# BDMstudio/audio-cut

Measured on AMD Instinct MI355X. Metric: audio-seconds processed/sec (separate+detect) per GPU; cut-point index parity, higher is better.
Workload: dtype f32

## Files before the change

### audio_cut_amd/csrc/ac_mdx.hip

```cpp
#include <math.h>

#include "ac_common.h"
#include "../../include/audiocut_hip_stereo.h"

#define MDX_NFFT 6144
#define MDX_M 3072
#define MDX_HOP 1024
#define MDX_T 256
#define MDX_F 3072
#define MDX_ITEM 261120
#define MDX_TRIM 3072
#define MDX_GEN 254976

__device__ inline float2 cmulf(float2 a, float2 b) { return make_float2(a.x * b.x - a.y * b.y, a.x * b.y + a.y * b.x); }

__device__ inline float2 tw3072(const float2* __restrict__ tw, int q) {
    int k = 2 * q;
    if (k >= MDX_M) { const float2 t = tw[k - MDX_M]; return make_float2(-t.x, -t.y); }
    return tw[k];
}

__device__ float2* fft3072_f32(float2* a, float2* b, const float2* __restrict__ tw) {
    int Ns = 1;
    for (int pass = 0; pass < 5; ++pass) {
        for (int j = threadIdx.x; j < MDX_M / 4; j += 256) {
            const int k = j & (Ns - 1);
            float2 v0 = a[j], v1 = a[j + MDX_M / 4], v2 = a[j + MDX_M / 2], v3 = a[j + 3 * MDX_M / 4];
            if (Ns > 1) {
                const int q = k * (MDX_M / (4 * Ns));
                v1 = cmulf(v1, tw3072(tw, q));
                v2 = cmulf(v2, tw3072(tw, 2 * q));
                v3 = cmulf(v3, tw3072(tw, 3 * q));
            }
            const float2 s02 = make_float2(v0.x + v2.x, v0.y + v2.y), d02 = make_float2(v0.x - v2.x, v0.y - v2.y);
            const float2 s13 = make_float2(v1.x + v3.x, v1.y + v3.y), d13 = make_float2(v1.x - v3.x, v1.y - v3.y);
            const int base = ((j - k) << 2) + k;
            b[base] = make_float2(s02.x + s13.x, s02.y + s13.y);
            b[base + Ns] = make_float2(d02.x + d13.y, d02.y - d13.x);
            b[base + 2 * Ns] = make_float2(s02.x - s13.x, s02.y - s13.y);
            b[base + 3 * Ns] = make_float2(d02.x - d13.y, d02.y + d13.x);
        }
        __syncthreads();
        float2* t = a; a = b; b = t;
        Ns <<= 2;
    }
    {
        const float c3 = -0.5f, s3 = -0.86602540378443864676f;
        for (int j = threadIdx.x; j < MDX_M / 3; j += 256) {
            const int k = j;
            float2 v0 = a[j], v1 = a[j + 1024], v2 = a[j + 2048];
            v1 = cmulf(v1, tw3072(tw, k));
            v2 = cmulf(v2, tw3072(tw, 2 * k));
            const float2 s = make_float2(v1.x + v2.x, v1.y + v2.y);
            const float2 d = make_float2(v1.x - v2.x, v1.y - v2.y);
            const float2 m = make_float2(v0.x + c3 * s.x, v0.y + c3 * s.y);
            const float2 r = make_float2(-s3 * d.y, s3 * d.x);
            b[k] = make_float2(v0.x + s.x, v0.y + s.y);
            b[k + 1024] = make_float2(m.x + r.x, m.y + r.y);
            b[k + 2048] = make_float2(m.x - r.x, m.y - r.y);
        }
        __syncthreads();
        float2* t = a; a = b; b = t;
    }
    return a;
}

template <int CH>
__global__ __launch_bounds__(256) void k_mdx_stft(const float* __restrict__ track, int64_t n,
                                                  const int64_t* __restrict__ chunk_start,
                                                  const int64_t* __restrict__ chunk_len,
                                                  const int32_t* __restrict__ win_index,
                                                  const float2* __restrict__ tw, const float* __restrict__ hann,
                                                  float* __restrict__ spec, float* __restrict__ spec_amax) {
    __shared__ float2 s_a[MDX_M];
    __shared__ float2 s_b[MDX_M];
    const int t = blockIdx.x;
    const int item = blockIdx.y;
    const int ch = CH == 2 ? (int)blockIdx.z : 0;
    const float* x = track + (size_t)ch * n;
    const int64_t cs = chunk_start[item];
    const int64_t cl = chunk_len[item];
    const int64_t woff = (int64_t)win_index[item] * MDX_GEN - MDX_TRIM;
    for (int m = threadIdx.x; m < MDX_M; m += 256) {
        float v[2];
#pragma unroll
        for (int h = 0; h < 2; ++h) {
            const int i = 2 * m + h;
            int jj = t * MDX_HOP - MDX_NFFT / 2 + i;
            if (jj < 0) jj = -jj;
            else if (jj >= MDX_ITEM) jj = 2 * (MDX_ITEM - 1) - jj;
            const int64_t q = woff + jj;
            const float s = (q >= 0 && q < cl) ? x[cs + q] : 0.f;
            v[h] = s * hann[i];
        }
        s_a[m] = make_float2(v[0], v[1]);
    }
    __syncthreads();
    const float2* Z = fft3072_f32(s_a, s_b, tw);
    const size_t cstride = (size_t)MDX_T * MDX_F;
    float* out = spec + (size_t)item * 4 * cstride + 2 * ch * cstride + (size_t)t * MDX_F;
    float vmax = 0.f;
    for (int k = threadIdx.x; k < MDX_F; k += 256) {
        const float2 zk = Z[k];
        const float2 zn = Z[(MDX_M - k) % MDX_M];
        const float2 e = make_float2(0.5f * (zk.x + zn.x), 0.5f * (zk.y - zn.y));
        const float2 o = make_float2(0.5f * (zk.x - zn.x), 0.5f * (zk.y + zn.y));
        const float2 wo = cmulf(tw[k], o);
        const float re = e.x + wo.y, im = e.y - wo.x;
        out[k] = re;
        out[cstride + k] = im;
        if (CH == 1) {
            out[2 * cstride + k] = re;
            out[3 * cstride + k] = im;
        }
        vmax = fmaxf(vmax, fmaxf(fabsf(re), fabsf(im)));
    }
    if (spec_amax) ac_amax_commit(vmax, spec_amax + (size_t)item * MDX_T + t);
}

extern "C" int ac_mdx_stft(ac_ctx* ctx, const float* track, int64_t n, const int64_t* chunk_start, const int64_t* chunk_len,
                           const int32_t* win_index, int n_items, float* spec_out, float* spec_amax, void* stream) {
    AC_REQUIRE(ctx && track && chunk_start && chunk_len && win_index && spec_out, "null pointer");
    AC_REQUIRE(n > 0 && n_items > 0 && n_items <= 65535, "n_items must be in [1, 65535]");
    hipLaunchKernelGGL(k_mdx_stft<1>, dim3(MDX_T, n_items), dim3(256), 0, (hipStream_t)stream, track, n, chunk_start, chunk_len,
                       win_index, ctx->tw6144, ctx->hann6144, spec_out, spec_amax);
    AC_LAUNCH_CHECK();
    return AC_OK;
}

extern "C" int ac_mdx_stft_stereo(ac_ctx* ctx, const float* track, int64_t n, const int64_t* chunk_start, const int64_t* chunk_len,
                                  const int32_t* win_index, int n_items, float* spec_out, float* spec_amax, void* stream) {
    AC_REQUIRE(ctx && track && chunk_start && chunk_len && win_index && spec_out, "null pointer");
    AC_REQUIRE(n > 0 && n_items > 0 && n_items <= 65535, "n_items must be in [1, 65535]");
    hipLaunchKernelGGL(k_mdx_stft<2>, dim3(MDX_T, n_items, 2), dim3(256), 0, (hipStream_t)stream, track, n, chunk_start, chunk_len,
                       win_index, ctx->tw6144, ctx->hann6144, spec_out, spec_amax);
    AC_LAUNCH_CHECK();
    return AC_OK;
}

__global__ __launch_bounds__(256) void k_mdx_istft_frames(const float* __restrict__ spec, const float2* __restrict__ tw,
                                                          const float* __restrict__ hann, float* __restrict__ frames) {
    __shared__ float2 s_a[MDX_M];
    __shared__ float2 s_b[MDX_M];
    const int t = blockIdx.x, ch = blockIdx.y, item = blockIdx.z;
    const size_t cstride = (size_t)MDX_T * MDX_F;
    const float* re_p = spec + ((size_t)item * 4 + 2 * ch) * cstride + (size_t)t * MDX_F;
    const float* im_p = re_p + cstride;
    for (int k = threadIdx.x; k < MDX_M; k += 256) {
        float2 xk = make_float2(re_p[k], k == 0 ? 0.f : im_p[k]);
        float2 xm = (k == 0) ? make_float2(0.f, 0.f) : make_float2(re_p[MDX_M - k], im_p[MDX_M - k]);
        const float2 e = make_float2(0.5f * (xk.x + xm.x), 0.5f * (xk.y - xm.y));
        const float2 d = make_float2(0.5f * (xk.x - xm.x), 0.5f * (xk.y + xm.y));
        const float2 w = tw[k];
        const float2 o = cmulf(make_float2(w.x, -w.y), d);
        s_a[k] = make_float2(e.x - o.y, -(e.y + o.x));
    }
    __syncthreads();
    const float2* z = fft3072_f32(s_a, s_b, tw);
    const float inv = 1.0f / (float)MDX_M;
    float* out = frames + (((size_t)item * 2 + ch) * MDX_T + t) * MDX_NFFT;
    for (int m = threadIdx.x; m < MDX_M; m += 256) {
        const float2 v = z[m];
        const float x0 = v.x * inv, x1 = -v.y * inv;
        const float2 hw = reinterpret_cast<const float2*>(hann)[m];
        reinterpret_cast<float2*>(out)[m] = make_float2(x0 * hw.x, x1 * hw.y);
    }
}

__global__ __launch_bounds__(256) void k_mdx_istft_ola(const float* __restrict__ frames, const float* __restrict__ env,
                                                       float* __restrict__ wave) {
    const int64_t idx = (int64_t)blockIdx.x * 256 + threadIdx.x;
    const int64_t row = idx / MDX_ITEM;
    const int nn = (int)(idx - row * MDX_ITEM);
    const int p = nn + MDX_NFFT / 2;
    int t_lo = (p - (MDX_NFFT - 1) + MDX_HOP - 1) / MDX_HOP;
    if (p - (MDX_NFFT - 1) <= 0) t_lo = 0;
    int t_hi = p / MDX_HOP;
    if (t_hi > MDX_T - 1) t_hi = MDX_T - 1;
    const float* base = frames + (size_t)row * MDX_T * MDX_NFFT;
    float acc = 0.f;
    for (int t = t_lo; t <= t_hi; ++t) acc += base[(size_t)t * MDX_NFFT + (p - t * MDX_HOP)];
    wave[idx] = acc / env[p];
}

extern "C" int ac_mdx_istft(ac_ctx* ctx, const float* spec, int n_items, float* wave_out, float* scratch, void* stream) {
    AC_REQUIRE(ctx && spec && wave_out && scratch, "null pointer");
    AC_REQUIRE(n_items > 0 && n_items <= 65535, "n_items must be in [1, 65535]");
    hipLaunchKernelGGL(k_mdx_istft_frames, dim3(MDX_T, 2, n_items), dim3(256), 0, (hipStream_t)stream, spec, ctx->tw6144,
                       ctx->hann6144, scratch);
    AC_LAUNCH_CHECK();
    const int64_t total = (int64_t)n_items * 2 * MDX_ITEM;
    hipLaunchKernelGGL(k_mdx_istft_ola, dim3((unsigned)(total / 256)), dim3(256), 0, (hipStream_t)stream, scratch,
                       ctx->ola_env6144, wave_out);
    AC_LAUNCH_CHECK();
    return AC_OK;
}

template <int CH>
__global__ __launch_bounds__(256) void k_mdx_assemble_ola(const float* __restrict__ track, int64_t n, const float* __restrict__ wave,
                                                          const int64_t* __restrict__ chunk_start,
                                                          const int64_t* __restrict__ chunk_len,
                                                          const int64_t* __restrict__ eff_start,
                                                          const int64_t* __restrict__ eff_end,
                                                          const int32_t* __restrict__ item_base, int n_chunks,
                                                          float* __restrict__ vocal_out, float* __restrict__ inst_out,
                                                          float* __restrict__ vocal_st_out, float* __restrict__ inst_st_out) {
    const int64_t g = (int64_t)blockIdx.x * 256 + threadIdx.x;
    if (g >= n) return;
    int lo = 0, hi = n_chunks;
    while (lo < hi) { const int mid = (lo + hi) >> 1; if (eff_end[mid] > g) hi = mid; else lo = mid + 1; }
    const int c_lo = lo;
    const float m0 = track[g];
    const float m1 = CH == 2 ? track[n + g] : m0;
    float v_acc = 0.f, i_acc = 0.f, w_acc = 0.f;
    float v0_acc = 0.f, v1_acc = 0.f, i0_acc = 0.f, i1_acc = 0.f;
    for (int c = c_lo; c < n_chunks && eff_start[c] <= g; ++c) {
        if (eff_end[c] <= g) continue;
        const int64_t q = g - chunk_start[c];
        if (q < 0 || q >= chunk_len[c]) continue;
        const int item = item_base[c] + (int)(q / MDX_GEN);
        const int pos = MDX_TRIM + (int)(q % MDX_GEN);
        const float w0 = wave[((size_t)item * 2 + 0) * MDX_ITEM + pos];
        const float w1 = wave[((size_t)item * 2 + 1) * MDX_ITEM + pos];
        const float vocal = (w0 + w1) * 0.5f;
        const float inst = ((m0 - w0) + (m1 - w1)) * 0.5f;
        v_acc += vocal;
        i_acc += inst;
        w_acc += 1.0f;
        if (CH == 2) {
            v0_acc += w0; v1_acc += w1;
            i0_acc += m0 - w0; i1_acc += m1 - w1;
        }
    }
    if (w_acc == 0.f) w_acc = 1.0f;
    vocal_out[g] = v_acc / w_acc;
    inst_out[g] = i_acc / w_acc;
    if (CH == 2) {
        if (vocal_st_out) { vocal_st_out[g] = v0_acc / w_acc; vocal_st_out[n + g] = v1_acc / w_acc; }
        if (inst_st_out) { inst_st_out[g] = i0_acc / w_acc; inst_st_out[n + g] = i1_acc / w_acc; }
    }
}

extern "C" int ac_mdx_assemble_ola(ac_ctx* ctx, const float* track, int64_t n, const float* wave, const int64_t* chunk_start,
                                   const int64_t* chunk_len, const int64_t* eff_start, const int64_t* eff_end,
                                   const int32_t* item_base, int n_chunks, float* vocal_out, float* inst_out, void* stream) {
    AC_REQUIRE(ctx && track && wave && chunk_start && chunk_len && eff_start && eff_end && item_base && vocal_out && inst_out,
               "null pointer");
    AC_REQUIRE(n > 0 && n_chunks > 0, "sizes must be positive");
    const int64_t blocks = (n + 255) / 256;
    AC_REQUIRE(blocks < (1LL << 31), "track too long");
    hipLaunchKernelGGL(k_mdx_assemble_ola<1>, dim3((unsigned)blocks), dim3(256), 0, (hipStream_t)stream, track, n, wave, chunk_start,
                       chunk_len, eff_start, eff_end, item_base, n_chunks, vocal_out, inst_out, nullptr, nullptr);
    AC_LAUNCH_CHECK();
    return AC_OK;
}

extern "C" int ac_mdx_assemble_ola_stereo(ac_ctx* ctx, const float* track, int64_t n, const float* wave, const int64_t* chunk_start,
                                          const int64_t* chunk_len, const int64_t* eff_start, const int64_t* eff_end,
                                          const int32_t* item_base, int n_chunks, float* vocal_out, float* inst_out,
                                          float* vocal_st_out, float* inst_st_out, void* stream) {
    AC_REQUIRE(ctx && track && wave && chunk_start && chunk_len && eff_start && eff_end && item_base && vocal_out && inst_out,
               "null pointer");
    AC_REQUIRE(n > 0 && n_chunks > 0, "sizes must be positive");
    const int64_t blocks = (n + 255) / 256;
    AC_REQUIRE(blocks < (1LL << 31), "track too long");
    hipLaunchKernelGGL(k_mdx_assemble_ola<2>, dim3((unsigned)blocks), dim3(256), 0, (hipStream_t)stream, track, n, wave, chunk_start,
                       chunk_len, eff_start, eff_end, item_base, n_chunks, vocal_out, inst_out, vocal_st_out, inst_st_out);
    AC_LAUNCH_CHECK();
    return AC_OK;
}

template <int CH>
__global__ __launch_bounds__(256) void k_mdx_chunk_vocal(const float* __restrict__ track, int64_t n, const float* __restrict__ wave,
                                                         const int64_t* __restrict__ chunk_start,
                                                         const int64_t* __restrict__ chunk_len,
                                                         const int64_t* __restrict__ out_offset,
                                                         const int32_t* __restrict__ item_base, int mix_minus,
                                                         float* __restrict__ out) {
    const int c = blockIdx.y;
    const int64_t cl = chunk_len[c];
    const int64_t cs = CH == 2 ? chunk_start[c] : 0;
    float* dst = out + out_offset[c];
    for (int64_t q = (int64_t)blockIdx.x * 256 + threadIdx.x; q < cl; q += (int64_t)gridDim.x * 256) {
        const int item = item_base[c] + (int)(q / MDX_GEN);
        const int pos = MDX_TRIM + (int)(q % MDX_GEN);
        const float w0 = wave[((size_t)item * 2 + 0) * MDX_ITEM + pos];
        const float w1 = wave[((size_t)item * 2 + 1) * MDX_ITEM + pos];
        if (CH == 2 && mix_minus) dst[q] = ((track[cs + q] - w0) + (track[n + cs + q] - w1)) * 0.5f;
        else dst[q] = (w0 + w1) * 0.5f;
    }
}

extern "C" int ac_mdx_chunk_vocal(ac_ctx* ctx, const float* wave, const int64_t* chunk_len, const int64_t* out_offset,
                                  const int32_t* item_base, int n_chunks, float* out, void* stream) {
    AC_REQUIRE(ctx && wave && chunk_len && out_offset && item_base && out, "null pointer");
    AC_REQUIRE(n_chunks > 0 && n_chunks <= 65535, "n_chunks must be in [1, 65535]");
    hipLaunchKernelGGL(k_mdx_chunk_vocal<1>, dim3(256, n_chunks), dim3(256), 0, (hipStream_t)stream, nullptr, (int64_t)0, wave,
                       nullptr, chunk_len, out_offset, item_base, 0, out);
    AC_LAUNCH_CHECK();
    return AC_OK;
}

extern "C" int ac_mdx_chunk_vocal_stereo(ac_ctx* ctx, const float* track, int64_t n, const float* wave, const int64_t* chunk_start,
                                         const int64_t* chunk_len, const int64_t* out_offset, const int32_t* item_base, int n_chunks,
                                         int mix_minus, float* out, void* stream) {
    AC_REQUIRE(ctx && wave && chunk_start && chunk_len && out_offset && item_base && out, "null pointer");
    AC_REQUIRE(!mix_minus || (track && n > 0), "mix_minus needs the track");
    AC_REQUIRE(n_chunks > 0 && n_chunks <= 65535, "n_chunks must be in [1, 65535]");
    hipLaunchKernelGGL(k_mdx_chunk_vocal<2>, dim3(256, n_chunks), dim3(256), 0, (hipStream_t)stream, track, n, wave, chunk_start,
                       chunk_len, out_offset, item_base, mix_minus, out);
    AC_LAUNCH_CHECK();
    return AC_OK;
}

extern "C" int ac_stereo_abi_version(void) { return AC_STEREO_ABI_VERSION; }

__global__ __launch_bounds__(256) void k_sum_squares(const float* __restrict__ x, int64_t n, double* __restrict__ out) {
    __shared__ double s_red[4];
    double acc = 0.0;
    for (int64_t i = (int64_t)blockIdx.x * 256 + threadIdx.x; i < n; i += (int64_t)gridDim.x * 256) { const double v = x[i]; acc += v * v; }
    const double tot = block_sum_f64_256(acc, s_red);
    if (threadIdx.x == 0) out[blockIdx.x] = tot;
}

__global__ __launch_bounds__(256) void k_window_sum_squares(const float* __restrict__ x, const int64_t* __restrict__ w_start,
                                                            const int64_t* __restrict__ w_end, double* __restrict__ out) {
    __shared__ double s_red[4];
    const int64_t a = w_start[blockIdx.x], b = w_end[blockIdx.x];
    double acc = 0.0;
    for (int64_t i = a + threadIdx.x; i < b; i += 256) { const double v = x[i]; acc += v * v; }
    const double tot = block_sum_f64_256(acc, s_red);
    if (threadIdx.x == 0) out[blockIdx.x] = tot;
}

extern "C" int ac_window_sum_squares(ac_ctx* ctx, const float* x, int64_t n, const int64_t* w_start, const int64_t* w_end, int n_windows,
                                     double* out, void* stream) {
    AC_REQUIRE(ctx && x && w_start && w_end && out, "null pointer");
    AC_REQUIRE(n > 0 && n_windows > 0, "sizes must be positive");
    hipLaunchKernelGGL(k_window_sum_squares, dim3((unsigned)n_windows), dim3(256), 0, (hipStream_t)stream, x, w_start, w_end, out);
    AC_LAUNCH_CHECK();
    return AC_OK;
}

extern "C" int ac_sum_squares(ac_ctx* ctx, const float* x, int64_t n, double* partials, int n_partials, void* stream) {
    AC_REQUIRE(ctx && x && partials, "null pointer");
    AC_REQUIRE(n > 0 && n_partials > 0 && n_partials <= 4096, "n_partials must be in [1, 4096]");
    hipLaunchKernelGGL(k_sum_squares, dim3(n_partials), dim3(256), 0, (hipStream_t)stream, x, n, partials);
    AC_LAUNCH_CHECK();
    return AC_OK;
}
```

Before: 1509.

## Fuse MDX iSTFT frame FFT with overlap-add, keeping frames in registers

Replaces the two-kernel iSTFT (per-frame inverse FFT written to a scratch frame buffer, then a gather-based overlap-add) with one kernel. Each workgroup handles a strip of hops, runs the frames' inverse FFTs with a new register-heavy radix-4/radix-3 FFT over padded LDS, and accumulates overlap-add sums in registers before writing normalized output. This removes the large scratch frame write/read and a launch. In exchange, neighbouring strips recompute up to five overlapping frames, and the heavier register use limits occupancy.

Result: no change. 1518, median of 6 (+0.6%).

```diff
diff --git a/audio_cut_amd/csrc/ac_mdx.hip b/audio_cut_amd/csrc/ac_mdx.hip
--- a/audio_cut_amd/csrc/ac_mdx.hip
+++ b/audio_cut_amd/csrc/ac_mdx.hip
@@ -138,60 +138,188 @@
     return AC_OK;
 }
 
-__global__ __launch_bounds__(256) void k_mdx_istft_frames(const float* __restrict__ spec, const float2* __restrict__ tw,
-                                                          const float* __restrict__ hann, float* __restrict__ frames) {
-    __shared__ float2 s_a[MDX_M];
-    __shared__ float2 s_b[MDX_M];
-    const int t = blockIdx.x, ch = blockIdx.y, item = blockIdx.z;
-    const size_t cstride = (size_t)MDX_T * MDX_F;
-    const float* re_p = spec + ((size_t)item * 4 + 2 * ch) * cstride + (size_t)t * MDX_F;
-    const float* im_p = re_p + cstride;
-    for (int k = threadIdx.x; k < MDX_M; k += 256) {
+__device__ inline float2 tw3072_sel(const float2* tw, unsigned q) {
+    const unsigned k = 2 * q;
+    const bool neg = k >= MDX_M;
+    const float2 t = tw[neg ? k - MDX_M : k];
+    return neg ? make_float2(-t.x, -t.y) : t;
+}
+
+__device__ inline void bfly4(float2 v0, float2 v1, float2 v2, float2 v3, float2& o0, float2& o1, float2& o2, float2& o3) {
+    const float2 s02 = make_float2(v0.x + v2.x, v0.y + v2.y), d02 = make_float2(v0.x - v2.x, v0.y - v2.y);
+    const float2 s13 = make_float2(v1.x + v3.x, v1.y + v3.y), d13 = make_float2(v1.x - v3.x, v1.y - v3.y);
+    o0 = make_float2(s02.x + s13.x, s02.y + s13.y);
+    o1 = make_float2(d02.x + d13.y, d02.y - d13.x);
+    o2 = make_float2(s02.x - s13.x, s02.y - s13.y);
+    o3 = make_float2(d02.x - d13.y, d02.y + d13.x);
+}
+
+#define MDX_LDS (MDX_M + MDX_M / 16)
+__device__ inline unsigned mdx_pad(unsigned x) { return x + (x >> 4); }
+static_assert(6 * MDX_LDS * sizeof(float2) <= 160 * 1024, "six workgroups of k_mdx_istft per CU by LDS (160 KiB); its registers admit four");
+
+template <class Load>
+__device__ inline void fft3072_paired(Load load, const unsigned tid, float2* s, const float2* tw) {
+    const unsigned k16 = tid & 15;
+    float2 x[16], w2[3], w3[4][3], w4[3], w5[4][2];
+    if (tid < 192) {
+        float2 y[16];
+#pragma unroll
+        for (int e = 0; e < 16; ++e) x[e] = load(tid + 192 * e);
+#pragma unroll
+        for (int i = 0; i < 4; ++i)
+            bfly4(x[i], x[i + 4], x[i + 8], x[i + 12], y[4 * i], y[4 * i + 1], y[4 * i + 2], y[4 * i + 3]);
+#pragma unroll
+        for (int m = 0; m < 4; ++m) {
+            const unsigned q = 192 * m;
+            bfly4(y[m], cmulf(y[4 + m], tw3072_sel(tw, q)), cmulf(y[8 + m], tw3072_sel(tw, 2 * q)), cmulf(y[12 + m], tw3072_sel(tw, 3 * q)),
+                  x[m], x[m + 4], x[m + 8], x[m + 12]);
+        }
+#pragma unroll
+        for (int m = 1; m < 4; ++m) {
+            w2[m - 1] = tw3072_sel(tw, 48 * k16 * m);
+#pragma unroll
+            for (int b = 0; b < 4; ++b) w3[b][m - 1] = tw3072_sel(tw, 12 * (k16 + 16 * b) * m);
+        }
+    }
+    __syncthreads();
+    if (tid < 192) {
+#pragma unroll
+        for (int e = 0; e < 16; ++e) s[17 * tid + e] = x[e];
+    }
+    __syncthreads();
+    if (tid < 192) {
+        float2 y[16];
+#pragma unroll
+        for (int e = 0; e < 16; ++e) x[e] = s[mdx_pad(tid + 192 * e)];
+#pragma unroll
+        for (int i = 0; i < 4; ++i)
+            bfly4(x[i], cmulf(x[i + 4], w2[0]), cmulf(x[i + 8], w2[1]), cmulf(x[i + 12], w2[2]),
+                  y[4 * i], y[4 * i + 1], y[4 * i + 2], y[4 * i + 3]);
+#pragma unroll
+        for (int m = 0; m < 4; ++m)
+            bfly4(y[m], cmulf(y[4 + m], w3[m][0]), cmulf(y[8 + m], w3[m][1]), cmulf(y[12 + m], w3[m][2]),
+                  x[m], x[m + 4], x[m + 8], x[m + 12]);
+    }
+#pragma unroll
+    for (int m = 1; m < 4; ++m) w4[m - 1] = tw3072_sel(tw, 3 * tid * m);
+    __syncthreads();
+    if (tid < 192) {
+#pragma unroll
+        for (int e = 0; e < 16; ++e) s[16 * (tid - k16) + k16 + 16 * e] = x[e];
+    }
+    __syncthreads();
+#pragma unroll
+    for (int r = 0; r < 3; ++r) {
+        const unsigned j = tid + 256 * r;
+        bfly4(s[j], cmulf(s[j + MDX_M / 4], w4[0]), cmulf(s[j + MDX_M / 2], w4[1]), cmulf(s[j + 3 * MDX_M / 4], w4[2]),
+              x[4 * r], x[4 * r + 1], x[4 * r + 2], x[4 * r + 3]);
+    }
+#pragma unroll
+    for (int r = 0; r < 4; ++r) {
+        w5[r][0] = tw3072_sel(tw, tid + 256 * r);
+        w5[r][1] = tw3072_sel(tw, 2 * (tid + 256 * r));
+    }
+    __syncthreads();
+#pragma unroll
+    for (int e = 0; e < 12; ++e) s[1024 * (e >> 2) + tid + 256 * (e & 3)] = x[e];
+    __syncthreads();
+    const float c3 = -0.5f, s3 = -0.86602540378443864676f;
+#pragma unroll
+    for (int r = 0; r < 4; ++r) {
+        const unsigned k = tid + 256 * r;
+        const float2 v0 = s[k], v1 = cmulf(s[k + 1024], w5[r][0]), v2 = cmulf(s[k + 2048], w5[r][1]);
+        const float2 sm = make_float2(v1.x + v2.x, v1.y + v2.y);
+        const float2 d = make_float2(v1.x - v2.x, v1.y - v2.y);
+        const float2 m = make_float2(v0.x + c3 * sm.x, v0.y + c3 * sm.y);
+        const float2 rr = make_float2(-s3 * d.y, s3 * d.x);
+        x[3 * r] = make_float2(v0.x + sm.x, v0.y + sm.y);
+        x[3 * r + 1] = make_float2(m.x + rr.x, m.y + rr.y);
+        x[3 * r + 2] = make_float2(m.x - rr.x, m.y - rr.y);
+    }
+    __syncthreads();
+#pragma unroll
+    for (int r = 0; r < 4; ++r) {
+        const unsigned k = tid + 256 * r;
+        s[k] = x[3 * r]; s[k + 1024] = x[3 * r + 1]; s[k + 2048] = x[3 * r + 2];
+    }
+    __syncthreads();
+}
+
+__device__ inline void mdx_istft_frame(const float* __restrict__ re_p, const float* __restrict__ im_p, const unsigned tid, float2* s,
+                                       const float2* tw) {
+    fft3072_paired([&](unsigned k) {
         float2 xk = make_float2(re_p[k], k == 0 ? 0.f : im_p[k]);
         float2 xm = (k == 0) ? make_float2(0.f, 0.f) : make_float2(re_p[MDX_M - k], im_p[MDX_M - k]);
         const float2 e = make_float2(0.5f * (xk.x + xm.x), 0.5f * (xk.y - xm.y));
         const float2 d = make_float2(0.5f * (xk.x - xm.x), 0.5f * (xk.y + xm.y));
-        const float2 w = tw[k];
-        const float2 o = cmulf(make_float2(w.x, -w.y), d);
-        s_a[k] = make_float2(e.x - o.y, -(e.y + o.x));
-    }
-    __syncthreads();
-    const float2* z = fft3072_f32(s_a, s_b, tw);
+        const float2 wk = tw[k];
+        const float2 o = cmulf(make_float2(wk.x, -wk.y), d);
+        return make_float2(e.x - o.y, -(e.y + o.x));
+    }, tid, s, tw);
+}
+
+#define MDX_OLA_G 16
+__global__ __launch_bounds__(256, 4) void k_mdx_istft(const float* __restrict__ spec, const float2* tw,
+                                                   const float* hann, const float* __restrict__ env,
+                                                   float* __restrict__ wave) {
+    __shared__ float2 s_z[MDX_LDS];
+    unsigned tid = threadIdx.x;
+    const int ch = blockIdx.y, item = blockIdx.z;
+    const int hp0 = 3 + MDX_OLA_G * (int)blockIdx.x;
+    const int hp1 = hp0 + MDX_OLA_G < MDX_T + 2 ? hp0 + MDX_OLA_G : MDX_T + 2;
+    const int t0 = hp0 - 5 > 0 ? hp0 - 5 : 0;
+    const int t1 = hp1 - 1 < MDX_T - 1 ? hp1 - 1 : MDX_T - 1;
+    const size_t cstride = (size_t)MDX_T * MDX_F;
+    const float* re_c = spec + ((size_t)item * 4 + 2 * ch) * cstride;
+    const float2* hann2 = reinterpret_cast<const float2*>(hann);
+    const float2* env2 = reinterpret_cast<const float2*>(env);
+    float2* out = reinterpret_cast<float2*>(wave + ((size_t)item * 2 + ch) * MDX_ITEM);
     const float inv = 1.0f / (float)MDX_M;
-    float* out = frames + (((size_t)item * 2 + ch) * MDX_T + t) * MDX_NFFT;
-    for (int m = threadIdx.x; m < MDX_M; m += 256) {
-        const float2 v = z[m];
-        const float x0 = v.x * inv, x1 = -v.y * inv;
-        const float2 hw = reinterpret_cast<const float2*>(hann)[m];
-        reinterpret_cast<float2*>(out)[m] = make_float2(x0 * hw.x, x1 * hw.y);
-    }
-}
-
-__global__ __launch_bounds__(256) void k_mdx_istft_ola(const float* __restrict__ frames, const float* __restrict__ env,
-                                                       float* __restrict__ wave) {
-    const int64_t idx = (int64_t)blockIdx.x * 256 + threadIdx.x;
-    const int64_t row = idx / MDX_ITEM;
-    const int nn = (int)(idx - row * MDX_ITEM);
-    const int p = nn + MDX_NFFT / 2;
-    int t_lo = (p - (MDX_NFFT - 1) + MDX_HOP - 1) / MDX_HOP;
-    if (p - (MDX_NFFT - 1) <= 0) t_lo = 0;
-    int t_hi = p / MDX_HOP;
-    if (t_hi > MDX_T - 1) t_hi = MDX_T - 1;
-    const float* base = frames + (size_t)row * MDX_T * MDX_NFFT;
-    float acc = 0.f;
-    for (int t = t_lo; t <= t_hi; ++t) acc += base[(size_t)t * MDX_NFFT + (p - t * MDX_HOP)];
-    wave[idx] = acc / env[p];
+    float2 acc[6][2];
+#pragma unroll
+    for (int s = 0; s < 6; ++s) acc[s][0] = acc[s][1] = make_float2(0.f, 0.f);
+    auto emit = [&](const float2 (&a)[2], int hp) {
+#pragma unroll
+        for (int u = 0; u < 2; ++u) {
+            const unsigned pp = 512 * hp + 256 * u + tid;
+            const float2 ev = env2[pp];
+            out[pp - MDX_NFFT / 4] = make_float2(a[u].x / ev.x, a[u].y / ev.y);
+        }
+    };
+    for (int t = t0; t <= t1; ++t) {
+        asm volatile("" : "+v"(tid));
+        const float* re_p = re_c + (size_t)t * MDX_F;
+        mdx_istft_frame(re_p, re_p + cstride, tid, s_z, tw);
+#pragma unroll
+        for (int s = 0; s < 6; ++s) {
+            if (t + s < hp0 || t + s >= hp1) continue;
+#pragma unroll
+            for (int u = 0; u < 2; ++u) {
+                const unsigned m = 512 * s + 256 * u + tid;
+                const float2 v = s_z[m];
+                const float x0 = v.x * inv, x1 = -v.y * inv;
+                const float2 hw = hann2[m];
+                acc[s][u].x += x0 * hw.x;
+                acc[s][u].y += x1 * hw.y;
+            }
+        }
+        if (t >= hp0) emit(acc[0], t);
+        if (t == MDX_T - 1) {
+            if (hp0 <= MDX_T && MDX_T < hp1) emit(acc[1], MDX_T);
+            if (hp0 <= MDX_T + 1 && MDX_T + 1 < hp1) emit(acc[2], MDX_T + 1);
+        }
+#pragma unroll
+        for (int s = 0; s < 5; ++s) { acc[s][0] = acc[s + 1][0]; acc[s][1] = acc[s + 1][1]; }
+        acc[5][0] = acc[5][1] = make_float2(0.f, 0.f);
+    }
 }
 
 extern "C" int ac_mdx_istft(ac_ctx* ctx, const float* spec, int n_items, float* wave_out, float* scratch, void* stream) {
     AC_REQUIRE(ctx && spec && wave_out && scratch, "null pointer");
     AC_REQUIRE(n_items > 0 && n_items <= 65535, "n_items must be in [1, 65535]");
-    hipLaunchKernelGGL(k_mdx_istft_frames, dim3(MDX_T, 2, n_items), dim3(256), 0, (hipStream_t)stream, spec, ctx->tw6144,
-                       ctx->hann6144, scratch);
-    AC_LAUNCH_CHECK();
-    const int64_t total = (int64_t)n_items * 2 * MDX_ITEM;
-    hipLaunchKernelGGL(k_mdx_istft_ola, dim3((unsigned)(total / 256)), dim3(256), 0, (hipStream_t)stream, scratch,
-                       ctx->ola_env6144, wave_out);
+    hipLaunchKernelGGL(k_mdx_istft, dim3((MDX_T - 1 + MDX_OLA_G - 1) / MDX_OLA_G, 2, n_items), dim3(256), 0, (hipStream_t)stream,
+                       spec, ctx->tw6144, ctx->hann6144, ctx->ola_env6144, wave_out);
     AC_LAUNCH_CHECK();
     return AC_OK;
 }
```
